# kasvii/GATOR

Hardware: AMD Instinct MI355X
Metric: meshes/sec (B=256, J=17) GATOR forward (higher is better)
Workload: dtype f32; 1 GPU; B=256 synthetic Human3.6M 17-joint poses per GPU, GAT+MDR forward fp32; batch_per_gpu=256, global_batch=256, num_joint=17, impl=fused, parallelism=dp1, mode=gather

## Files before the change

gator_amd/csrc/fused_common.h:

```cpp
#pragma once
#include <hip/hip_runtime.h>

namespace gator {

typedef float f32x16 __attribute__((ext_vector_type(16)));
typedef float f32x4 __attribute__((ext_vector_type(4)));

#define GATOR_MFMA(a, b, c) __builtin_amdgcn_mfma_f32_32x32x2f32((a), (b), (c), 0, 0, 0)

__device__ __forceinline__ int kap(int r) { return (r & 3) + 8 * (r >> 2); }

__device__ __forceinline__ f32x16 zero16() {
    f32x16 z;
#pragma unroll
    for (int r = 0; r < 16; ++r) z[r] = 0.f;
    return z;
}

struct HalfPair { float lo, hi; };
__device__ __forceinline__ HalfPair xhalves(float v) {
    const unsigned u = __float_as_uint(v);
    const auto r = __builtin_amdgcn_permlane32_swap(u, u, false, false);
    return HalfPair{__uint_as_float(r[0]), __uint_as_float(r[1])};
}
__device__ __forceinline__ float xhalf(float v) {
    const HalfPair q = xhalves(v);
    return (threadIdx.x & 32) ? q.lo : q.hi;
}

struct WTile { f32x4 g[4]; };

__device__ __forceinline__ WTile load_wtile(const float* __restrict__ Wp, int tile, int lane) {
    const f32x4* p = reinterpret_cast<const f32x4*>(Wp) + ((size_t)tile * 4) * 64 + lane;
    WTile t;
#pragma unroll
    for (int g = 0; g < 4; ++g) t.g[g] = p[g * 64];
    return t;
}

__device__ __forceinline__ f32x16 mma_T(const WTile& w, const f32x16& x, f32x16 acc) {
#pragma unroll
    for (int g = 0; g < 4; ++g)
#pragma unroll
        for (int j = 0; j < 4; ++j) acc = GATOR_MFMA(w.g[g][j], x[4 * g + j], acc);
    return acc;
}
__device__ __forceinline__ f32x16 mma_C(const WTile& w, const f32x16& x, f32x16 acc) {
#pragma unroll
    for (int g = 0; g < 4; ++g)
#pragma unroll
        for (int j = 0; j < 4; ++j) acc = GATOR_MFMA(x[4 * g + j], w.g[g][j], acc);
    return acc;
}

__device__ __forceinline__ void mma2_T(const WTile& w0, const f32x16& x0, f32x16& a0, const WTile& w1, const f32x16& x1, f32x16& a1) {
#pragma unroll
    for (int g = 0; g < 4; ++g)
#pragma unroll
        for (int j = 0; j < 4; ++j) {
            a0 = GATOR_MFMA(w0.g[g][j], x0[4 * g + j], a0);
            a1 = GATOR_MFMA(w1.g[g][j], x1[4 * g + j], a1);
        }
}
__device__ __forceinline__ void mma2_C(const WTile& w0, const f32x16& x0, f32x16& a0, const WTile& w1, const f32x16& x1, f32x16& a1) {
#pragma unroll
    for (int g = 0; g < 4; ++g)
#pragma unroll
        for (int j = 0; j < 4; ++j) {
            a0 = GATOR_MFMA(x0[4 * g + j], w0.g[g][j], a0);
            a1 = GATOR_MFMA(x1[4 * g + j], w1.g[g][j], a1);
        }
}
__device__ __forceinline__ f32x16 dot16(const f32x16& A, const f32x16& B, f32x16 init) {
    f32x16 e = init, o = zero16();
#pragma unroll
    for (int r = 0; r < 16; r += 2) {
        e = GATOR_MFMA(A[r], B[r], e);
        o = GATOR_MFMA(A[r + 1], B[r + 1], o);
    }
    return e + o;
}
__device__ __forceinline__ void dot16x2(const f32x16& A0, const f32x16& B0, f32x16& a0, const f32x16& A1, const f32x16& B1, f32x16& a1) {
#pragma unroll
    for (int r = 0; r < 16; ++r) {
        a0 = GATOR_MFMA(A0[r], B0[r], a0);
        a1 = GATOR_MFMA(A1[r], B1[r], a1);
    }
}

__device__ __forceinline__ f32x16 load_chanvec_T(const float* __restrict__ vec, int base, int h) {
    f32x16 v;
#pragma unroll
    for (int g = 0; g < 4; ++g) {
// ... 169 lines not shown
```

gator_amd/csrc/mdr_fused.hip:

```cpp
#include "fused_common.h"
#include "fused_state.h"
#include "x3_common.h"

#include <cmath>
#include <cstddef>
#include <cstdlib>
#include <type_traits>

namespace gator {
namespace {

constexpr float kLog2e = 1.4426950408889634f;

#ifdef GATOR_DIAG
__device__ int g_mdr_wmask = -1, g_mdr_kvmask = -1;
__device__ unsigned long long* g_persist_ends = nullptr;
#define MDR_WIDX(i) ((i) & g_mdr_wmask)
#define MDR_KVIDX(i) ((i) & g_mdr_kvmask)
#else
#define MDR_WIDX(i) (i)
#define MDR_KVIDX(i) (i)
#endif

struct LayerW {
// ... 136 lines not shown
    float m = -1e30f, l = 0.f;
    const float c = kLog2e * 0.17677669529663688110f;
#pragma unroll 1
    for (int kt = 0; kt < kVT - 2; kt += 4) {
        {
            const f32x16 kb = load_block(kbase + (size_t)kt * 2 * kTile, lane), vb = load_block(vbase + (size_t)kt * 2 * kTile, lane);
            ATTN_TILE(kt, kb, vb, O, O2)
        }
        {
            const f32x16 kb = load_block(kbase + (size_t)(kt + 1) * 2 * kTile, lane), vb = load_block(vbase + (size_t)(kt + 1) * 2 * kTile, lane);
            ATTN_TILE(kt + 1, kb, vb, O3, O4)
        }
        {
            const f32x16 kb = load_block(kbase + (size_t)(kt + 2) * 2 * kTile, lane), vb = load_block(vbase + (size_t)(kt + 2) * 2 * kTile, lane);
            ATTN_TILE(kt + 2, kb, vb, O, O2)
        }
        {
            const f32x16 kb = load_block(kbase + (size_t)(kt + 3) * 2 * kTile, lane), vb = load_block(vbase + (size_t)(kt + 3) * 2 * kTile, lane);
            ATTN_TILE(kt + 3, kb, vb, O3, O4)
        }
    }
    {
        const f32x16 kb = load_block(kbase + (size_t)(kVT - 2) * 2 * kTile, lane), vb = load_block(vbase + (size_t)(kVT - 2) * 2 * kTile, lane);
        ATTN_TILE(kVT - 2, kb, vb, O, O2)
    }
    {
        const f32x16 kb = load_block(kbase + (size_t)(kVT - 1) * 2 * kTile, lane), vb = load_block(vbase + (size_t)(kVT - 1) * 2 * kTile, lane);
        ATTN_TILE(kVT - 1, kb, vb, O3, O4)
    }
    l += xhalf(l);
    return ((O + O2) + (O3 + O4)) * (1.0f / l);
}

#define ATTN_TILE_X3(KT, KB, VB, OACC)                                                                      \
    {                                                                                                       \
        f32x16 S = x3_mma(KB, qx, zero16());                                           \
        float bm = -1e30f;                                                                                  \
        _Pragma("unroll") for (int r = 0; r < 16; ++r) {    \
            float sc = S[r];                                                                                \
            if ((KT) == kVT - 1 && kap(r) + 4 * h >= kV - 32 * (kVT - 1)) sc = -1e30f;                      \
            S[r] = sc;                                                                                      \
            bm = fmaxf(bm, sc);                                                                             \
        }                                                                                                   \
        bm = fmaxf(bm, xhalf(bm));                                                                          \
        if (!__all(bm <= m + 8.0f)) {                                                                       \
            const float mn = fmaxf(m, bm);                                                                  \
            const float al = __builtin_amdgcn_exp2f(m - mn);                                                \
            O = O * al;                                                                                     \
            O2 = O2 * al;                                                                                   \
            l *= al;                                                                                        \
            m = mn;                                                                                         \
        }                                                                                                   \
        float ps = 0.f;                                                                                     \
        _Pragma("unroll") for (int r = 0; r < 16; ++r) {                                                    \
            const float pe = __builtin_amdgcn_exp2f(S[r] - m);                                              \
            S[r] = pe;                                                                                      \
            ps += pe;                                                                                       \
        }                                                                                                   \
        l += ps;                                                                                            \
        OACC = x3_mma(VB, x3_split(S), OACC);             \
    }
__device__ __forceinline__ f32x16 self_attention_head_x3(const float* __restrict__ qt, const float* __restrict__ kbase,
                                                         const float* __restrict__ vbase, int lane) {
    const int h = lane >> 5;
    const X3 qx = x3_load(qt, lane);
    f32x16 O = zero16(), O2 = zero16();
    float m = -1e30f, l = 0.f;
    X3 kb = x3_load(kbase, lane), vb = x3_load(vbase, lane);
#pragma unroll 1
    for (int kt = 0; kt < kVT; kt += 2) {
        X3 kn = x3_load(kbase + (size_t)(kt + 1) * 2 * kTileX3, lane), vn = x3_load(vbase + (size_t)(kt + 1) * 2 * kTileX3, lane);
        ATTN_TILE_X3(kt, kb, vb, O)
        const int k2 = kt + 2 < kVT ? kt + 2 : kt;
        kb = x3_load(kbase + (size_t)k2 * 2 * kTileX3, lane);
        vb = x3_load(vbase + (size_t)k2 * 2 * kTileX3, lane);
        ATTN_TILE_X3(kt + 1, kn, vn, O2)
    }
    l += xhalf(l);
    return (O + O2) * (1.0f / l);
}

constexpr float kX2QK = 16.0f, kX2V = 16.0f;
#define ATTN_PV(VB, PX) { O2 = x2_mma_small(VB, PX, O2); O = x2_mma_main(VB, PX, O); }
#define ATTN_TILE_X2(KT, KB, VB)                                                                            \
    {                                                                                                       \
        MDR_PRIO_MFMA();                                                                                    \
        f32x16 S = x2_mma(KB, qx, zero16());                                     \
        MDR_PRIO_VALU();                                                                                    \
        float bm = -1e30f;                                                                                  \
        _Pragma("unroll") for (int r = 0; r < 16; ++r) {                                                    \
            float sc = S[r];                                                                                \
            if ((KT) == kVT - 1 && kap(r) + 4 * h >= kV - 32 * (kVT - 1)) sc = -1e30f;                      \
            S[r] = sc;                                                                                      \
            bm = fmaxf(bm, sc);                                                                             \
        }                                                                                                   \
        bm = fmaxf(bm, xhalf(bm));                                                                          \
        if (!__all(bm <= m + 2048.0f)) {                     \
            const float mn = fmaxf(m, bm);                                                                  \
            const float al = __builtin_amdgcn_exp2f((m - mn) * 0.00390625f);                                \
            O = O * al;                                                                                     \
            O2 = O2 * al;                                                                                   \
            l *= al;                                                                                        \
            m = mn;                                                                                         \
        }                                                                                                   \
        const float off = 6.0f - m * 0.00390625f;                                                           \
        float ps = 0.f;                                                                                     \
        _Pragma("unroll") for (int r = 0; r < 16; ++r) {                                                    \
            const float pe = __builtin_amdgcn_exp2f(fmaf(S[r], 0.00390625f, off));                          \
            S[r] = pe;                                                                                      \
            ps += pe;                                                                                       \
        }                                                                                                   \
        l += ps;                                                                                            \
        const X2 px_ = x2_split(S);                                                                         \
        MDR_PRIO_MFMA();                                                                                    \
                           \
        ATTN_PV(VB, px_)                                                                                    \
    }
template <bool kActScale16>
__device__ __forceinline__ f32x16 self_attention_head_x2(const float* __restrict__ qt, const float* __restrict__ kbase,
                                                         const float* __restrict__ vbase, int lane) {
    const int h = lane >> 5;
    const X2 qx = x2_load(qt, lane);
    f32x16 O = zero16(), O2 = zero16();
    float m = -1e30f, l = 0.f;
    X2 kb = x2_load(kbase, lane), vb = x2_load(vbase, lane);
#pragma unroll 1
    for (int kt = 0; kt < kVT - 2; kt += 2) {
        X2 kn = x2_load(kbase + (size_t)MDR_KVIDX(kt + 1) * 2 * kTile, lane), vn = x2_load(vbase + (size_t)MDR_KVIDX(kt + 1) * 2 * kTile, lane);
        ATTN_TILE_X2(0, kb, vb)
        kb = x2_load(kbase + (size_t)MDR_KVIDX(kt + 2) * 2 * kTile, lane);
        vb = x2_load(vbase + (size_t)MDR_KVIDX(kt + 2) * 2 * kTile, lane);
        ATTN_TILE_X2(0, kn, vn)
    }
    {
        X2 kn = x2_load(kbase + (size_t)MDR_KVIDX(kVT - 1) * 2 * kTile, lane), vn = x2_load(vbase + (size_t)MDR_KVIDX(kVT - 1) * 2 * kTile, lane);
        ATTN_TILE_X2(kVT - 2, kb, vb)
        ATTN_TILE_X2(kVT - 1, kn, vn)
    }
    l += xhalf(l);
    return (O + O2) * (((kActScale16 ? 16.0f : 1.0f) / kX2V) / l);
}


constexpr int kTileX1 = kTile / 2;
template <bool kActScale16>
__device__ __forceinline__ f32x16 self_attention_head_x1(const float* __restrict__ qt, const float* __restrict__ kbase,
                                                         const float* __restrict__ vbase, int lane) {
    const int h = lane >> 5;
    const X1 qx = x1_load(qt, lane);
    f32x16 O = zero16();
    float m = -1e30f, l = 0.f;
    X1 kA = x1_load(kbase, lane), vA = x1_load(vbase, lane);
    X1 kB = x1_load(kbase + (size_t)MDR_KVIDX(1) * 2 * kTileX1, lane), vB = x1_load(vbase + (size_t)MDR_KVIDX(1) * 2 * kTileX1, lane);
    f32x16 SA = x1_mma(kA, qx, zero16()), SB;
    float ci = 1e30f;
    auto step = [&](auto last_, const int kt, f32x16& Sc, f32x16& Sn, X1& Kc, const X1& Kn, X1& Vc) {
        constexpr int KT = decltype(last_)::value;
        if (KT != kVT - 1) Sn = x1_mma(Kn, qx, zero16());
        if (KT == kVT - 1) {
#pragma unroll
            for (int r = 0; r < 16; ++r) if (kap(r) + 4 * h >= kV - 32 * (kVT - 1)) Sc[r] = -1e30f;
        }
        float ps = 0.f;
        if (__all(ci < 1e29f)) {
#pragma unroll
            for (int r = 0; r < 16; ++r) { const float pe = __builtin_amdgcn_exp2f(Sc[r] + ci); ps += pe; Sc[r] = pe; }
        } else ps = 1e30f;
        if (!__all(ps < 32768.0f)) {
            f32x16 R = x1_mma(Kc, qx, zero16());
            float bm = -1e30f;
#pragma unroll
            for (int r = 0; r < 16; ++r) {
                if (KT == kVT - 1 && kap(r) + 4 * h >= kV - 32 * (kVT - 1)) R[r] = -1e30f;
                bm = fmaxf(bm, R[r]);
            }
            bm = fmaxf(bm, xhalf(bm));
            const float mn = fmaxf(m, bm);
            const float al = __builtin_amdgcn_exp2f(m - mn);
            O = O * al;
            l *= al;
            m = mn;
            ci = 6.0f - m;
            ps = 0.f;
#pragma unroll
            for (int r = 0; r < 16; ++r) { Sc[r] = __builtin_amdgcn_exp2f(R[r] + ci); ps += Sc[r]; }
        }
        l += ps;
        O = x1_mma(Vc, x1_cvt(Sc), O);
        __builtin_amdgcn_sched_barrier(0);
        if (kt + 2 < kVT) {
            Kc = x1_load(kbase + (size_t)MDR_KVIDX(kt + 2) * 2 * kTileX1, lane);
            Vc = x1_load(vbase + (size_t)MDR_KVIDX(kt + 2) * 2 * kTileX1, lane);
        }
        __builtin_amdgcn_sched_barrier(0);
    };
#pragma unroll 1
    for (int kt = 0; kt < kVT - 2; kt += 2) {
        step(std::integral_constant<int, 0>(), kt, SA, SB, kA, kB, vA);
        step(std::integral_constant<int, 0>(), kt + 1, SB, SA, kB, kA, vB);
    }
    step(std::integral_constant<int, 0>(), kVT - 2, SA, SB, kA, kB, vA);
    step(std::integral_constant<int, kVT - 1>(), kVT - 1, SB, SA, kB, kA, vB);
    l += xhalf(l);
    return O * (((kActScale16 ? 16.0f : 1.0f) / kX2V) / l);
}

__device__ __forceinline__ f32x16 cross_attention_head(const float* __restrict__ kj, const float* __restrict__ vjp,
                                                       const f32x16& qh, int J, int lane) {
    const int h = lane >> 5;
    const f32x16 kb = load_block(kj, lane);
    f32x16 S = dot16(kb, qh, zero16());
    const float c = kLog2e * 0.17677669529663688110f;
    float mx = -1e30f;
#pragma unroll
    for (int r = 0; r < 16; ++r) {
        const float s = (kap(r) + 4 * h < J) ? S[r] * c : -1e30f;
        S[r] = s;
        mx = fmaxf(mx, s);
    }
    mx = fmaxf(mx, xhalf(mx));
// ... 949 lines not shown
        float acc[3][3];
#pragma unroll
        for (int q = 0; q < 3; ++q) acc[q][0] = acc[q][1] = acc[q][2] = 0.f;
        int cch = lane / 3, ktap = lane - 3 * cch;
#pragma unroll(HOIST ? NIT : 1)
        for (int it = 0; it < NIT; ++it) {
            const int e = lane + 64 * it;
            if (e < kV * 3) {
                const float in0 = bn[cch][ktap], in1 = bn[cch][ktap + 1], in2 = bn[cch][ktap + 2];
#pragma unroll
                for (int q = 0; q < 3; ++q) {
                    const float w = HOIST ? wreg[q][HOIST ? it : 0] : conv_w(q, it);
                    acc[q][0] = fmaf(w, in0, acc[q][0]);
                    acc[q][1] = fmaf(w, in1, acc[q][1]);
                    acc[q][2] = fmaf(w, in2, acc[q][2]);
                }
            }
            cch += ktap == 2 ? 22 : 21;
            ktap = ktap == 2 ? 0 : ktap + 1;
        }
#pragma unroll
        for (int q = 0; q < 3; ++q)
#pragma unroll
            for (int l = 0; l < 3; ++l) {
                const double s = wave_sum64_f64((double)acc[q][l]);
                const int m = wave + NW * q;
                if (lane == 0 && m < 20) bc[m][l] = (float)(s + (double)a.bconv_b[m]);
            }
    }
    __syncthreads();
    const int mt = b >> 5, sl = b & 31;
    bool poisoned = false;
    if (a.persist_ctr) {
        int ch, b0, n;
        a.plan.locate(b, ch, b0, n);
        const unsigned* blk = a.persist_ctr + a.plan.block(ch);
        poisoned = blk[kCtrError] != 0u || blk[kCtrDone + (size_t)3 * n + (b - b0)] != (unsigned)kVT;
    }
    const float limit = a.vcp2 ? 4094.0f : 3.0e38f;
    bool bad = false;
    if (tok) {
        if (!HOIST) load_rows();
        float av[20];
#pragma unroll
        for (int g = 0; g < 5; ++g) { av[4 * g] = row[g][0]; av[4 * g + 1] = row[g][1]; av[4 * g + 2] = row[g][2]; av[4 * g + 3] = row[g][3]; }
        float mx = -1e30f, p[20], l = 0.f;
        for (int m = 0; m < 20; ++m) mx = fmaxf(mx, av[m]);
        for (int m = 0; m < 20; ++m) {
            p[m] = __builtin_amdgcn_exp2f((av[m] - mx) * kLog2e);
            l += p[m];
        }
        const float il = 1.0f / l;
        const float sc = a.alpha ? (float)exp((double)tail[3] * 0.09531017980432493) : 1.0f;
        const int cb = v >> 5, g = (v & 31) >> 3, hh = (v & 7) >> 2, j = v & 3;
        for (int c = 0; c < 3; ++c) {
            float o = 0.f;
            for (int m = 0; m < 20; ++m) o += (p[m] * il) * bc[m][c];
            float val = sc * o + cc[c];
            if (poisoned) val = __builtin_nanf("");
            bad = bad || !(fabsf(val) < limit);
            a.vc[((size_t)b * kV + v) * 3 + c] = val;
            if (a.vcp2) {
                const float sv = val * 16.0f;
                const _Float16 hi = (_Float16)sv;
                const _Float16 lo = (_Float16)(sv - (float)hi);
                const size_t pair = ((((size_t)(mt >> 2) * 28 + (v >> 4)) * 4 + (mt & 3)) * 3 + c) * 2;
                const size_t e = (size_t)(((v >> 3) & 1) * 32 + sl) * 8 + (v & 7);
                a.vcp2[pair * 512 + e] = hi; a.vcp2[(pair + 1) * 512 + e] = lo;
            } else if (a.vcp3) {
                const __bf16 hi = (__bf16)val;
                const float r1 = val - (float)hi;
                const __bf16 mid = (__bf16)r1;
                const __bf16 lo = (__bf16)(r1 - (float)mid);
                const size_t e = ((((size_t)mt * 3 + c) * 28 + (v >> 4)) * 64 + ((v >> 3) & 1) * 32 + sl) * 8 + (v & 7);
                a.vcp3[e] = hi; a.vcp3[a.vcp3_plane + e] = mid; a.vcp3[2 * a.vcp3_plane + e] = lo;
            } else {
                a.vcp[(((((size_t)mt * 3 + c) * kCB + cb) * 4 + g) * 64 + hh * 32 + sl) * 4 + j] = val;
            }
        }
    }
    head_report(a, b, bad, poisoned);
}

__global__ __launch_bounds__(256) void k_mdr_head_finish(const HeadArgs a, const double* __restrict__ hpart) {
    __shared__ float bc[20][3];
    const int b = blockIdx.x;
    bool poisoned = false;
    if (a.persist_ctr) {
        int ch, b0, n;
        a.plan.locate(b, ch, b0, n);
        const unsigned* blk = a.persist_ctr + a.plan.block(ch);
        poisoned = blk[kCtrError] != 0u || blk[kCtrDone + (size_t)3 * n + (b - b0)] != (unsigned)kVT;
    }
    head_finish<256>(a, hpart + (size_t)b * kVT * 64, b, poisoned, bc);
}

LayerW make_layer(const FusedState* f, const gator_ctx* c, int li) {
    const MdrLayerP& p = f->lay[li];
    const MdrLayerW& r = c->w.lay[li];
    LayerW w;
    auto sel = [&](const float* t) { return f->opt.mdr_x3 ? f->wxbuf + (size_t)(t - f->lay[0].wq) / kTile * kTileX3 : t; };
    w.wq = sel(p.wq); w.proj = sel(p.proj); w.fc1 = sel(p.fc1); w.fc2 = sel(p.fc2);
    w.sa0 = sel(p.sa[0]); w.sa1 = sel(p.sa[1]); w.sa2 = sel(p.sa[2]); w.sa3 = sel(p.sa[3]);
    w.n1w = r.n1w; w.n1b = r.n1b; w.proj_b = r.proj_b; w.n2w = r.n2w; w.n2b = r.n2b; w.fc1_b = r.fc1_b; w.fc2_b = r.fc2_b;
    w.a2 = r.a2; w.b2 = r.b2; w.sa0_b = r.sa_b[0]; w.sa1_b = r.sa_b[1]; w.sa2_b = r.sa_b[2]; w.sa3_b = r.sa_b[3];
    return w;
}

using MdrLayerKernel = void (*)(const MdrArgs, int);
using MdrPersistKernel = void (*)(const MdrPersistArgs);
constexpr MdrLayerKernel kMdrLayer[4][3] = {{k_mdr_layer<0, 3>, k_mdr_layer<1, 3>, k_mdr_layer<2, 3>}, {k_mdr_layer<0, 2>, k_mdr_layer<1, 2>, k_mdr_layer<2, 2>},
                                            {k_mdr_layer<0, 1>, k_mdr_layer<1, 1>, k_mdr_layer<2, 1>}, {k_mdr_layer<0, 0>, k_mdr_layer<1, 0>, k_mdr_layer<2, 0>}};
constexpr MdrPersistKernel kMdrPersist[4] = {k_mdr_persist<3>, k_mdr_persist<2>, k_mdr_persist<1>, k_mdr_persist<0>};

#ifdef GATOR_DIAG
struct MdrDiag { DevBuf<unsigned long long> st, ends; size_t solo = 0; };

int mdr_diag_setup(const FusedState* f, bool persist, hipStream_t st, MdrDiag& d) {
    static const int keep = -1, cut = 0;
    GATOR_HIP_CHECK(hipMemcpyToSymbolAsync(HIP_SYMBOL(g_mdr_wmask), (f->opt.mdr_cut & 1) ? &cut : &keep, sizeof(int), 0, hipMemcpyHostToDevice, st));
    GATOR_HIP_CHECK(hipMemcpyToSymbolAsync(HIP_SYMBOL(g_mdr_kvmask), (f->opt.mdr_cut & 2) ? &cut : &keep, sizeof(int), 0, hipMemcpyHostToDevice, st));
    d.solo = f->opt.mdr_solo ? 60 * 1024 : 0;
    if (f->opt.mdr_stamps) { GATOR_TRY(d.st.alloc(512 * sizeof(unsigned long long))); GATOR_HIP_CHECK(hipMemset(d.st, 0, 512 * sizeof(unsigned long long))); }
    if (f->opt.mdr_ends && persist) {
        GATOR_TRY(d.ends.alloc(3 * 1024 * sizeof(unsigned long long)));
        unsigned long long* d_ends = d.ends.get();
        GATOR_HIP_CHECK(hipMemset(d_ends, 0, 3 * 1024 * sizeof(unsigned long long)));
        GATOR_HIP_CHECK(hipMemcpyToSymbol(HIP_SYMBOL(g_persist_ends), &d_ends, sizeof(d_ends)));
    }
    return GATOR_OK;
}

int mdr_diag_report(MdrDiag& d, int B) {
    if (d.ends) {
        std::vector<unsigned long long> he(3 * 1024);
        GATOR_HIP_CHECK(hipMemcpy(he.data(), d.ends, he.size() * sizeof(unsigned long long), hipMemcpyDeviceToHost));
        unsigned long long* none = nullptr;
        GATOR_HIP_CHECK(hipMemcpyToSymbol(HIP_SYMBOL(g_persist_ends), &none, sizeof(none)));
        d.ends.reset();
        unsigned long long t0 = ~0ull, t1 = 0;
        int n = 0;
        for (int i = 0; i < 1024; ++i) if (he[3 * i + 2]) { t0 = std::min(t0, he[3 * i]); t1 = std::max(t1, he[3 * i + 2]); ++n; }
        if (n) {
            double idle = 0, lastlen = 0, first_end = 1e30, start_spread = 0;
            std::vector<double> ends;
            for (int i = 0; i < 1024; ++i) if (he[3 * i + 2]) {
                idle += (double)(t1 - he[3 * i + 2]) / 100.0;
                lastlen += (double)(he[3 * i + 2] - he[3 * i + 1]) / 100.0;
                first_end = std::min(first_end, (double)(he[3 * i + 2] - t0) / 100.0);
                start_spread = std::max(start_spread, (double)(he[3 * i] - t0) / 100.0);
                ends.push_back((double)(he[3 * i + 2] - t0) / 100.0);
            }
            std::sort(ends.begin(), ends.end());
            fprintf(stderr, "[k_mdr_persist ends, B=%d, %d workgroups] span %.1f us; workgroup starts spread over %.1f us; ends: first %.1f, p10 %.1f, median %.1f, p90 %.1f, last %.1f us; "
                            "mean idle before the last workgroup ends %.1f us; mean length of a workgroup's last stage-3 ticket %.1f us\n",
                    B, n, (double)(t1 - t0) / 100.0, start_spread, first_end, ends[n / 10], ends[n / 2], ends[n * 9 / 10], ends[n - 1], idle / n, lastlen / n);
        }
    }
    if (d.st) {
        unsigned long long hst[512];
        GATOR_HIP_CHECK(hipMemcpy(hst, d.st, sizeof(hst), hipMemcpyDeviceToHost));
        const int ns = (B * kVT + 63) / 64;
        unsigned long long t0 = ~0ull;
        for (int i = 0; i < ns && i < 120; ++i) if (hst[8 + 4 * i] && hst[8 + 4 * i] < t0) t0 = hst[8 + 4 * i];
        fprintf(stderr, "[k_mdr_layer<1> timeline, every 64th tile: tile:(start_us end_us kcycles xcc cu)]");
        for (int i = 0; i < ns && i < 120; ++i)
            fprintf(stderr, " %d:(%.0f,%.0f,%llu,x%llu,cu%llu.se%llu)", i * 64, (hst[8 + 4 * i] - t0) / 100.0, (hst[9 + 4 * i] - t0) / 100.0,
                    hst[10 + 4 * i] / 1000, hst[11 + 4 * i] >> 32, (hst[11 + 4 * i] >> 8) & 0xf, (hst[11 + 4 * i] >> 13) & 0x7);
        fprintf(stderr, "\n");
        d.st.reset();
        fprintf(stderr, "[k_mdr_layer<1> stamps, tile 0] attention(2 heads)=%llu outproj+res=%llu cross-attn block=%llu mlp=%llu customLN+qkv=%llu\n",
                hst[0], hst[1], hst[2], hst[3], hst[4]);
    }
    return GATOR_OK;
}
#endif

// ... 9 lines not shown
    ja.mdr_ctr = p.ctr_zero == CtrZero::MDR_JOINT ? ws.mdr_ctr : nullptr;
    ja.x2 = f->opt.mdr_x3 == 2;
    if (pc) {
        StageTimer tm(c, "mdr_joint", stream);
        k_mdr_joint<<<B, 128, 0, st>>>(ja);
    }
    const size_t per = (size_t)ws.cap * kVT * 2 * kTile;
    const size_t perq = (size_t)ws.cap * kVT * 2 * (f->opt.mdr_x3 == 1 ? kTileX3 : kTile);
    float* set[3][4] = {{ws.vf, ws.q, ws.k, ws.v}, {ws.vf + per, ws.q + perq, ws.k + perq, ws.v + perq},
                        {ws.vf + 2 * per, ws.q + 2 * perq, ws.k + 2 * perq, ws.v + 2 * perq}};
    MdrArgs a{};
    a.B = B; a.J = c->J; a.jkv = ws.jkv; a.pc = pc; a.xout = pc ? nullptr : x_out; a.vj = w.vj; a.tok_base = f->tok_base; a.tok_w3 = f->tok_w3;
    a.head_w = f->opt.mdr_x3 ? f->wxbuf + (size_t)(f->head_w - f->lay[0].wq) / kTile * kTileX3 : f->head_w; a.head_b = f->head_b; a.hf = ws.hf; a.lbf = c->block_taps ? ws.lbf : nullptr;
    a.hpart = p.head == MdrHead::FINISH ? reinterpret_cast<double*>(ws.hpart) : nullptr;
    a.bconv_w = w.bconv_w; a.hbn_w = w.bn_w; a.hbn_b = w.bn_b; a.hbn_mean = w.bn_mean; a.hbn_var = w.bn_var; a.halpha = c->alpha;
    a.lin_s = f->opt.mdr_x3 == 2 ? std::ldexp(kActScale, f->mdr_wshift) : 1.0f;
    a.lin_inv = 1.0f / a.lin_s;
    const int nwg = (B * kVT + 3) / 4;
#ifdef GATOR_DIAG
    MdrDiag diag;
    GATOR_TRY(mdr_diag_setup(f, persist, st, diag));
    const size_t solo = xa != 0 ? diag.solo : 0;
#else
    constexpr size_t solo = 0;
#endif
    MdrPersistArgs pa{};
    for (int li = 0; li <= 3; ++li) {
#ifdef GATOR_DIAG
        a.stamps = (li == 1) ? diag.st.get() : nullptr;
#endif
        float** in = persist ? set[(li + 2) % 3] : set[(li + 1) & 1];
        float** out = persist ? set[li % 3] : set[li & 1];
        a.layer = li;
        a.vf_in = in[0]; a.q_in = in[1]; a.k_in = in[2]; a.v_in = in[3];
        a.vf_out = out[0]; a.q_out = out[1]; a.k_out = out[2]; a.v_out = out[3];
        if (li > 0) a.prev = make_layer(f, c, li - 1);
        if (li < 3) a.cur = make_layer(f, c, li);
        if (persist) { pa.st[li] = a; continue; }
        StageTimer tm(c, li == 0 ? "mdr_layer0" : (li < 3 ? "mdr_layer" : "mdr_attn_head"), stream);
        const MdrLayerKernel layer = kMdrLayer[3 - xa][li == 0 ? 0 : li < 3 ? 1 : 2];
        layer<<<nwg, 256, li < 3 ? solo : 0, st>>>(a, nwg);
    }
    if (persist) {
        StageTimer tm(c, "mdr_layers", stream);
        const size_t tq = f->opt.mdr_x3 == 1 ? kTileX3 : (xa == 3 ? kTileX1 : kTile);
        for (int ch = 0, b0 = 0; ch < p.chunks.nch; ++ch) {
            const int n = p.chunks.base + (ch < p.chunks.rem ? 1 : 0);
            MdrPersistArgs pc_ = pa;
            for (int li = 0; li <= 3; ++li) {
                MdrArgs& s = pc_.st[li];
                const size_t ov = (size_t)b0 * kVT * 2 * kTile, oq = (size_t)b0 * kVT * 2 * tq;
                s.B = n;
                s.vf_in += ov; s.q_in += oq; s.k_in += oq; s.v_in += oq;
                s.vf_out += ov; s.q_out += oq; s.k_out += oq; s.v_out += oq;
                s.jkv += (size_t)b0 * 12 * kTile;
                if (s.pc) s.pc += (size_t)b0 * c->J * 133;
                if (s.xout) s.xout += (size_t)b0 * c->J * 3;
                s.hf += (size_t)b0 * kV * 32;
                if (s.hpart) s.hpart += (size_t)b0 * kVT * 64;
                if (s.lbf) s.lbf += (size_t)b0 * kV * kE;
            }
            pc_.ctr = ws.mdr_ctr + p.chunks.block(ch);
            const MdrPersistKernel layers = kMdrPersist[3 - xa];
            layers<<<p.grid, 256, 0, st>>>(pc_);
            b0 += n;
        }
    }
#ifdef GATOR_DIAG
    GATOR_TRY(mdr_diag_report(diag, B));
#endif
    HeadArgs ha;
    ha.hf = ws.hf; ha.bn_w = w.bn_w; ha.bn_b = w.bn_b; ha.bn_mean = w.bn_mean; ha.bn_var = w.bn_var;
    ha.bconv_w = w.bconv_w; ha.bconv_b = w.bconv_b; ha.vc = ws.vc; ha.vcp = ws.vcp;
    ha.persist_ctr = persist ? ws.mdr_ctr : nullptr;
    ha.plan = p.chunks;
    ha.status = c->status_dev;
    ha.pose2d = pose2d; ha.J = c->J;
    ha.vcp2 = f->opt.up_x3 == 2 ? (_Float16*)ws.vcp3 : nullptr;
    ha.vcp3 = f->opt.up_x3 == 1 ? (__bf16*)ws.vcp3 : nullptr; ha.vcp3_plane = upsample_x3_vcp_elems(ws.cap) / 3;
    ha.alpha = c->alpha;
    {
        StageTimer tm(c, "mdr_head", stream);
        switch (p.head) {
        case MdrHead::FINISH: k_mdr_head_finish<<<B, 256, 0, st>>>(ha, a.hpart); break;
        case MdrHead::WHOLE_HOIST: k_mdr_head<512, true><<<B, 512, 0, st>>>(ha); break;
        case MdrHead::WHOLE: k_mdr_head<512, false><<<B, 512, 0, st>>>(ha); break;
        }
    }
    GATOR_HIP_CHECK(hipGetLastError());
    c->set_tap(TAP_MDR_LBF2, c->block_taps ? ws.lbf : nullptr, c->block_taps ? (int64_t)B * kV * kE : 0);
    c->set_tap(TAP_VERT431, ws.vc, (int64_t)B * kV * 3);
    return GATOR_OK;
}

}
```

gator_amd/csrc/upsample_x2.hip:

```cpp
#include <cmath>
#include <cstring>

#include "upsample_common.h"

namespace gator {
namespace {

constexpr int kNBuf = 4, kStageFrags = 36;
constexpr int kActShift = 4;

__device__ __forceinline__ void split2(float x, _Float16& h, _Float16& l) {
    h = (_Float16)x;
    l = (_Float16)(x - (float)h);
}

__global__ void k_pack_up_x2(const float* __restrict__ w, _Float16* __restrict__ dst, int64_t n_frag_pairs, float scale) {
    const int64_t e = (int64_t)blockIdx.x * blockDim.x + threadIdx.x;
    if (e >= n_frag_pairs * 512) return;
    const int j = e & 7, lane = (e >> 3) & 63;
    int64_t r = e >> 9;
    const int tap = r % 3; r /= 3;
    const int o2 = r & 1; r >>= 1;
    const int s = r % kS16;
    const int op = (int)(r / kS16);
    const int o = 32 * (2 * op + o2) + (lane & 31), c = 16 * s + 8 * (lane >> 5) + j;
    const float x = (o < kNV && c < kV) ? w[((int64_t)o * kV + c) * 3 + tap] * scale : 0.f;
    _Float16 h, l;
    split2(x, h, l);
    const int64_t pair = (((int64_t)op * kS16 + s) * 2 + o2) * 3 + tap;
    dst[(pair * 2 + 0) * 512 + lane * 8 + j] = h;
    dst[(pair * 2 + 1) * 512 + lane * 8 + j] = l;
}
__global__ void k_pack_vc_x2(const float* __restrict__ vc, int B, _Float16* __restrict__ ap, int64_t n_frag_pairs) {
    const int64_t e = (int64_t)blockIdx.x * blockDim.x + threadIdx.x;
    if (e >= n_frag_pairs * 512) return;
    const int j = e & 7, lane = (e >> 3) & 63;
    int64_t r = e >> 9;
    const int lp = r % 3; r /= 3;
    const int mi = r & 3; r >>= 2;
    const int s = r % kS16;
    const int mg = (int)(r / kS16);
    const int smp = 32 * (4 * mg + mi) + (lane & 31), c = 16 * s + 8 * (lane >> 5) + j;
    const float x = (smp < B && c < kV) ? vc[((int64_t)smp * kV + c) * 3 + lp] * (float)(1 << kActShift) : 0.f;
    _Float16 h, l;
    split2(x, h, l);
    const int64_t pair = (((int64_t)mg * kS16 + s) * 4 + mi) * 3 + lp;
    ap[(pair * 2 + 0) * 512 + lane * 8 + j] = h;
    ap[(pair * 2 + 1) * 512 + lane * 8 + j] = l;
}

__global__ void k_absmax(const float* __restrict__ w, int64_t n, unsigned* __restrict__ out) {
    float m = 0.f;
    for (int64_t i = (int64_t)blockIdx.x * blockDim.x + threadIdx.x; i < n; i += (int64_t)gridDim.x * blockDim.x) {
        const float a = fabsf(w[i]);
        m = a > m || a != a ? a : m;
    }
    for (int o = 32; o > 0; o >>= 1) {
        const float q = __shfl_xor(m, o);
        m = q > m || q != q ? q : m;
    }
    if ((threadIdx.x & 63) == 0) atomicMax(out, __float_as_uint(m));
}

__device__ __forceinline__ void dma_frag(const void* base, unsigned lane_off, unsigned lds_dst) {
    unsigned keep;
    asm volatile("s_mov_b32 %0, m0\n\ts_mov_b32 m0, %3\n\ts_nop 0\n\tglobal_load_lds_dwordx4 %1, %2\n\ts_mov_b32 m0, %0"
                 : "=&s"(keep) : "v"(lane_off), "s"(base), "s"(lds_dst) : "memory");
}
template <int N> __device__ __forceinline__ void wait_vm() { asm volatile("s_waitcnt vmcnt(%0)" ::"n"(N) : "memory"); }

template <bool WLO = true>
__global__ __launch_bounds__(512, 1) void k_upsample_x2(const _Float16* __restrict__ ap, const _Float16* __restrict__ wp,
                                                        const float* __restrict__ bias, const float* __restrict__ tpl,
                                                        float* __restrict__ out, int B, int MT, int MG, int nwg, float unscale,
                                                        const JregEpi jr) {
    extern __shared__ __attribute__((aligned(16))) unsigned char lds_raw[];
    f16x8 (*st)[kStageFrags][64] = reinterpret_cast<f16x8 (*)[kStageFrags][64]>(lds_raw);
    const int lane = threadIdx.x & 63, wave = __builtin_amdgcn_readfirstlane(threadIdx.x >> 6);
    const int wg = xcd_remap(blockIdx.x, nwg);
    const int obp = wg / MG, mg = wg % MG;
    const int mi = wave & 3, oi = wave >> 2;
    const int ob = 2 * obp + oi, mt = 4 * mg + mi;
    const bool live = mt < MT;
    const unsigned lane_off = lane * 16;
    const unsigned lds0 = (unsigned)(unsigned long long)lds_raw;
    const char* a_src = reinterpret_cast<const char*>(ap) + (size_t)mg * kS16 * 24 * 1024;
    const char* w_src = reinterpret_cast<const char*>(wp) + (size_t)obp * kS16 * 12 * 1024;
    const char* src[5];
    unsigned stride[5], dsto[5];
#pragma unroll
    for (int i = 0; i < 5; ++i) {
        const int f = wave + 8 * i;
        src[i] = f < 24 ? a_src + f * 1024 : w_src + (f - 24) * 1024;
        stride[i] = f < 24 ? 24 * 1024 : 12 * 1024;
        dsto[i] = lds0 + f * 1024;
    }
    auto issue = [&](int s) {
        const unsigned dst = (unsigned)(s & (kNBuf - 1)) * kStageFrags * 1024;
#pragma unroll
        for (int i = 0; i < 4; ++i) dma_frag(src[i] + (size_t)s * stride[i], lane_off, dst + dsto[i]);
        if (wave < 4) dma_frag(src[4] + (size_t)s * stride[4], lane_off, dst + dsto[4]);
    };
    auto wait_landed = [&](int younger) {
        if (younger >= 1) { if (wave < 4) wait_vm<5>(); else wait_vm<4>(); }
        else wait_vm<0>();
    };
    f32x16 big[3], sm[3], tot[3];
#pragma unroll
    for (int l = 0; l < 3; ++l) { big[l] = zero16(); sm[l] = zero16(); tot[l] = zero16(); }
    f16x8 a[3][2], w[3][2];
    auto load_first = [&](int s) {
        const f16x8 (*cur)[64] = st[s & (kNBuf - 1)];
#pragma unroll
        for (int p = 0; p < 2; ++p) {
            a[0][p] = cur[mi * 6 + p][lane];
            w[0][p] = cur[24 + oi * 6 + p][lane];
            w[1][p] = cur[24 + oi * 6 + 2 + p][lane];
        }
    };
    auto load_rest = [&](int s) {
        const f16x8 (*cur)[64] = st[s & (kNBuf - 1)];
#pragma unroll
        for (int p = 0; p < 2; ++p) {
            a[1][p] = cur[mi * 6 + 2 + p][lane];
            w[2][p] = cur[24 + oi * 6 + 4 + p][lane];
            a[2][p] = cur[mi * 6 + 4 + p][lane];
        }
    };
    issue(0); issue(1); issue(2);
    if (wave < 4) wait_vm<10>(); else wait_vm<8>();
    __builtin_amdgcn_s_barrier();
    load_first(0);
#pragma unroll 1
    for (int s = 0; s < kS16; ++s) {
        if (s + 1 < kS16) wait_landed(kS16 - 2 - s);
        __builtin_amdgcn_s_barrier();
        if (s + 3 < kS16) issue(s + 3);
        load_rest(s);
        if (live) {
#pragma unroll
            for (int lp = 0; lp < 3; ++lp)
#pragma unroll
                for (int k = 2; k >= 0; --k) {
                    const int l = lp + 1 - k;
                    if (l < 0 || l > 2) continue;
                    big[l] = GATOR_MFMA_F16(a[lp][0], w[k][0], big[l]);
                    if constexpr (WLO) sm[l] = GATOR_MFMA_F16(a[lp][0], w[k][1], sm[l]);
                    sm[l] = GATOR_MFMA_F16(a[lp][1], w[k][0], sm[l]);
                }
            if (s % 7 == 6) {
#pragma unroll
                for (int l = 0; l < 3; ++l) { tot[l] += big[l]; big[l] = zero16(); }
            }
        }
        if (s + 1 < kS16) load_first(s + 1);
    }
    const int ov = 32 * ob + (lane & 31), h = lane >> 5;
    if (ov >= kNV || !live) return;
    const float bo = bias[ov];
    const float t0 = tpl[ov * 3], t1 = tpl[ov * 3 + 1], t2 = tpl[ov * 3 + 2];
    const int2 jb = jr.P ? jr.blk[ob] : int2{0, 0};
#pragma unroll
    for (int r = 0; r < 16; ++r) {
        const int smp = 32 * mt + kap(r) + 4 * h;
        if (smp < B) {
            F3 v;
            v.x = ((tot[0][r] + sm[0][r]) * unscale + bo) + t0;
            v.y = ((tot[1][r] + sm[1][r]) * unscale + bo) + t1;
            v.z = ((tot[2][r] + sm[2][r]) * unscale + bo) + t2;
            if (out) *reinterpret_cast<F3*>(out + ((int64_t)smp * kNV + ov) * 3) = v;
            for (int e = jb.x; e < jb.x + jb.y; ++e) {
                const int2 en = jr.ent[e];
                if (en.x == ov) {
                    const float we = jr.w[e];
                    F3 q;
                    q.x = we * v.x; q.y = we * v.y; q.z = we * v.z;
                    *reinterpret_cast<F3*>(jr.P + ((int64_t)smp * jr.nnz + en.y) * 3) = q;
                }
            }
        }
    }
}

constexpr size_t kX2Lds = (size_t)kNBuf * kStageFrags * 1024;

}

size_t upsample_x2_weight_elems() { return (size_t)(kOB / 2) * kS16 * 12 * 512; }
size_t upsample_x2_vcp_elems(int B) { return (size_t)((B + 127) / 128) * kS16 * 24 * 512; }

int upsample_x2_prepare_device() {
    GATOR_HIP_CHECK(hipFuncSetAttribute((const void*)k_upsample_x2<true>, hipFuncAttributeMaxDynamicSharedMemorySize, (int)kX2Lds));
    GATOR_HIP_CHECK(hipFuncSetAttribute((const void*)k_upsample_x2<false>, hipFuncAttributeMaxDynamicSharedMemorySize, (int)kX2Lds));
    return GATOR_OK;
}

int pack_upsample_x2(const float* up_w, void* dst, float* unscale, void* stream) {
    hipStream_t st = (hipStream_t)stream;
    DevBuf<unsigned> d_max;
    GATOR_TRY(d_max.alloc(sizeof(unsigned)));
    GATOR_HIP_CHECK(hipMemsetAsync(d_max, 0, sizeof(unsigned), st));
    const int64_t n = (int64_t)kNV * kV * 3;
    k_absmax<<<1024, 256, 0, st>>>(up_w, n, d_max.get());
    unsigned bits = 0;
    GATOR_HIP_CHECK(hipMemcpyAsync(&bits, d_max, sizeof(unsigned), hipMemcpyDeviceToHost, st));
    GATOR_HIP_CHECK(hipStreamSynchronize(st));
    d_max.reset();
    float wmax;
    static_assert(sizeof(wmax) == sizeof(bits), "float bits");
    memcpy(&wmax, &bits, sizeof(wmax));
    int shift = 0;
    if (wmax > 0.f && std::isfinite(wmax)) {
        int e;
        (void)std::frexp(wmax, &e);
        shift = 14 - e;
        if (shift > 118) shift = 118;
        if (shift < -118) shift = -118;
    }
    const int64_t pairs = (int64_t)upsample_x2_weight_elems() / 1024;
    k_pack_up_x2<<<(unsigned)((pairs * 512 + 255) / 256), 256, 0, st>>>(up_w, (_Float16*)dst, pairs, std::ldexp(1.0f, shift));
    GATOR_HIP_CHECK(hipGetLastError());
    *unscale = std::ldexp(1.0f, -(shift + kActShift));
    return GATOR_OK;
}

int launch_pack_vc_x2(const float* vc, int B, void* vcp2, void* stream) {
    const int64_t pairs = (int64_t)upsample_x2_vcp_elems(B) / 1024;
    k_pack_vc_x2<<<(unsigned)((pairs * 512 + 255) / 256), 256, 0, (hipStream_t)stream>>>(vc, B, (_Float16*)vcp2, pairs);
    GATOR_HIP_CHECK(hipGetLastError());
    return GATOR_OK;
}

int launch_upsample_x2(const FusedState* f, const gator_ctx* c, const FusedWs& ws, int B, float* verts, void* stream, bool with_joints, bool w1) {
    const int MT = (B + 31) / 32, MG = (MT + 3) / 4;
    const JregEpi jr = jreg_epi(f, with_joints);
    const int nwg = (kOB / 2) * MG;
    if (w1) k_upsample_x2<false><<<nwg, 512, kX2Lds, (hipStream_t)stream>>>((const _Float16*)ws.vcp3, (const _Float16*)f->up_w2.get(), c->w.up_b, c->w.v6890,
                                                                           verts, B, MT, MG, nwg, f->up_w2_unscale, jr);
// ... 8 lines not shown
```

Baseline: 447,200 meshes/sec.

## Trim masked work in last attention tile, skip padded upsample steps, widen head finish

The attention loop now gives the final key tile its own routine. It handles only the score registers that can hold live keys, and it issues three f16 MFMAs for PV instead of the full split product. The per-register mask check is removed from every other tile. The upsample GEMM loop now stops at the k-step count needed to cover the live columns rather than the padded kS16, with a final accumulation of the partial sums added. The head-finish kernel block size goes from 256 to 512 threads.

```diff
diff --git a/gator_amd/csrc/fused_common.h b/gator_amd/csrc/fused_common.h
--- a/gator_amd/csrc/fused_common.h
+++ b/gator_amd/csrc/fused_common.h
@@ -8,7 +8,7 @@
 
 #define GATOR_MFMA(a, b, c) __builtin_amdgcn_mfma_f32_32x32x2f32((a), (b), (c), 0, 0, 0)
 
-__device__ __forceinline__ int kap(int r) { return (r & 3) + 8 * (r >> 2); }
+__host__ __device__ __forceinline__ constexpr int kap(int r) { return (r & 3) + 8 * (r >> 2); }
 
 __device__ __forceinline__ f32x16 zero16() {
     f32x16 z;
diff --git a/gator_amd/csrc/mdr_fused.hip b/gator_amd/csrc/mdr_fused.hip
--- a/gator_amd/csrc/mdr_fused.hip
+++ b/gator_amd/csrc/mdr_fused.hip
@@ -242,18 +242,14 @@
 
 constexpr float kX2QK = 16.0f, kX2V = 16.0f;
 #define ATTN_PV(VB, PX) { O2 = x2_mma_small(VB, PX, O2); O = x2_mma_main(VB, PX, O); }
-#define ATTN_TILE_X2(KT, KB, VB)                                                                            \
+#define ATTN_TILE_X2(KB, VB)                                                                                \
     {                                                                                                       \
         MDR_PRIO_MFMA();                                                                                    \
         f32x16 S = x2_mma(KB, qx, zero16());                                     \
         MDR_PRIO_VALU();                                                                                    \
         float bm = -1e30f;                                                                                  \
-        _Pragma("unroll") for (int r = 0; r < 16; ++r) {                                                    \
-            float sc = S[r];                                                                                \
-            if ((KT) == kVT - 1 && kap(r) + 4 * h >= kV - 32 * (kVT - 1)) sc = -1e30f;                      \
-            S[r] = sc;                                                                                      \
-            bm = fmaxf(bm, sc);                                                                             \
-        }                                                                                                   \
+        _Pragma("unroll") for (int r = 0; r < 16; ++r)                                                      \
+            bm = fmaxf(bm, S[r]);                                                                           \
         bm = fmaxf(bm, xhalf(bm));                                                                          \
         if (!__all(bm <= m + 2048.0f)) {                     \
             const float mn = fmaxf(m, bm);                                                                  \
@@ -276,6 +272,53 @@
                            \
         ATTN_PV(VB, px_)                                                                                    \
     }
+constexpr int kLastTileKeys = kV - 32 * (kVT - 1);
+constexpr bool last_tile_kstep1_is_masked() {
+    for (int r = 8; r < 16; ++r)
+        if (kap(r) < kLastTileKeys) return false;
+    for (int r = 0; r < 8; ++r)
+        if (kap(r) + 4 >= 16) return false;
+    return true;
+}
+static_assert(kLastTileKeys > 0 && kLastTileKeys <= 16 && last_tile_kstep1_is_masked(),
+              "ATTN_TILE_X2_LAST skips score registers 8..15: every key they hold must be masked");
+#define ATTN_TILE_X2_LAST(KB, VB)                                                                           \
+    {                                                                                                       \
+        MDR_PRIO_MFMA();                                                                                    \
+        f32x16 S = x2_mma(KB, qx, zero16());                                                                \
+        MDR_PRIO_VALU();                                                                                    \
+        float bm = -1e30f;                                                                                  \
+        _Pragma("unroll") for (int r = 0; r < 8; ++r) {                                                     \
+            float sc = S[r];                                                                                \
+            if (kap(r) + 4 * h >= kLastTileKeys) sc = -1e30f;           \
+            S[r] = sc;                                                                                      \
+            bm = fmaxf(bm, sc);                                                                             \
+        }                                                                                                   \
+        bm = fmaxf(bm, xhalf(bm));                                                                          \
+        if (!__all(bm <= m + 2048.0f)) {                                                                    \
+            const float mn = fmaxf(m, bm);                                                                  \
+            const float al = __builtin_amdgcn_exp2f((m - mn) * 0.00390625f);                                \
+            O = O * al;                                                                                     \
+            O2 = O2 * al;                                                                                   \
+            l *= al;                                                                                        \
+            m = mn;                                                                                         \
+        }                                                                                                   \
+        const float off = 6.0f - m * 0.00390625f;                                                           \
+        float ps = 0.f;                                                                                     \
+        f16x8 ph_, pl_;                                                                                     \
+        _Pragma("unroll") for (int r = 0; r < 8; ++r) {                                                     \
+            const float pe = __builtin_amdgcn_exp2f(fmaf(S[r], 0.00390625f, off));                          \
+            ps += pe;                                                                                       \
+            const _Float16 hi_ = (_Float16)pe;                                      \
+            ph_[r] = hi_;                                                                                   \
+            pl_[r] = (_Float16)(pe - (float)hi_);                                                           \
+        }                                                                                                   \
+        l += ps;                                                                                            \
+        MDR_PRIO_MFMA();                                                                                    \
+        O2 = GATOR_MFMA_F16(VB.p[1][0], ph_, O2);                               \
+        O2 = GATOR_MFMA_F16(VB.p[0][0], pl_, O2);                                                           \
+        O = GATOR_MFMA_F16(VB.p[0][0], ph_, O);                                  \
+    }
 template <bool kActScale16>
 __device__ __forceinline__ f32x16 self_attention_head_x2(const float* __restrict__ qt, const float* __restrict__ kbase,
                                                          const float* __restrict__ vbase, int lane) {
@@ -287,15 +330,15 @@
 #pragma unroll 1
     for (int kt = 0; kt < kVT - 2; kt += 2) {
         X2 kn = x2_load(kbase + (size_t)MDR_KVIDX(kt + 1) * 2 * kTile, lane), vn = x2_load(vbase + (size_t)MDR_KVIDX(kt + 1) * 2 * kTile, lane);
-        ATTN_TILE_X2(0, kb, vb)
+        ATTN_TILE_X2(kb, vb)
         kb = x2_load(kbase + (size_t)MDR_KVIDX(kt + 2) * 2 * kTile, lane);
         vb = x2_load(vbase + (size_t)MDR_KVIDX(kt + 2) * 2 * kTile, lane);
-        ATTN_TILE_X2(0, kn, vn)
+        ATTN_TILE_X2(kn, vn)
     }
     {
         X2 kn = x2_load(kbase + (size_t)MDR_KVIDX(kVT - 1) * 2 * kTile, lane), vn = x2_load(vbase + (size_t)MDR_KVIDX(kVT - 1) * 2 * kTile, lane);
-        ATTN_TILE_X2(kVT - 2, kb, vb)
-        ATTN_TILE_X2(kVT - 1, kn, vn)
+        ATTN_TILE_X2(kb, vb)
+        ATTN_TILE_X2_LAST(kn, vn)
     }
     l += xhalf(l);
     return (O + O2) * (((kActScale16 ? 16.0f : 1.0f) / kX2V) / l);
@@ -1411,7 +1454,8 @@
     head_report(a, b, bad, poisoned);
 }
 
-__global__ __launch_bounds__(256) void k_mdr_head_finish(const HeadArgs a, const double* __restrict__ hpart) {
+constexpr int kHeadFinishNT = 512;
+__global__ __launch_bounds__(kHeadFinishNT) void k_mdr_head_finish(const HeadArgs a, const double* __restrict__ hpart) {
     __shared__ float bc[20][3];
     const int b = blockIdx.x;
     bool poisoned = false;
@@ -1421,7 +1465,7 @@
         const unsigned* blk = a.persist_ctr + a.plan.block(ch);
         poisoned = blk[kCtrError] != 0u || blk[kCtrDone + (size_t)3 * n + (b - b0)] != (unsigned)kVT;
     }
-    head_finish<256>(a, hpart + (size_t)b * kVT * 64, b, poisoned, bc);
+    head_finish<kHeadFinishNT>(a, hpart + (size_t)b * kVT * 64, b, poisoned, bc);
 }
 
 LayerW make_layer(const FusedState* f, const gator_ctx* c, int li) {
@@ -1597,7 +1641,7 @@
     {
         StageTimer tm(c, "mdr_head", stream);
         switch (p.head) {
-        case MdrHead::FINISH: k_mdr_head_finish<<<B, 256, 0, st>>>(ha, a.hpart); break;
+        case MdrHead::FINISH: k_mdr_head_finish<<<B, kHeadFinishNT, 0, st>>>(ha, a.hpart); break;
         case MdrHead::WHOLE_HOIST: k_mdr_head<512, true><<<B, 512, 0, st>>>(ha); break;
         case MdrHead::WHOLE: k_mdr_head<512, false><<<B, 512, 0, st>>>(ha); break;
         }
diff --git a/gator_amd/csrc/upsample_x2.hip b/gator_amd/csrc/upsample_x2.hip
--- a/gator_amd/csrc/upsample_x2.hip
+++ b/gator_amd/csrc/upsample_x2.hip
@@ -8,6 +8,9 @@
 
 constexpr int kNBuf = 4, kStageFrags = 36;
 constexpr int kActShift = 4;
+constexpr int kSteps = (kV + 15) / 16;
+static_assert(kSteps <= kS16 && 16 * kSteps >= kV, "every live column is inside a k-step that runs");
+static_assert(kSteps >= 3, "the prologue issues three stages");
 
 __device__ __forceinline__ void split2(float x, _Float16& h, _Float16& l) {
     h = (_Float16)x;
@@ -132,10 +135,10 @@
     __builtin_amdgcn_s_barrier();
     load_first(0);
 #pragma unroll 1
-    for (int s = 0; s < kS16; ++s) {
-        if (s + 1 < kS16) wait_landed(kS16 - 2 - s);
+    for (int s = 0; s < kSteps; ++s) {
+        if (s + 1 < kSteps) wait_landed(kSteps - 2 - s);
         __builtin_amdgcn_s_barrier();
-        if (s + 3 < kS16) issue(s + 3);
+        if (s + 3 < kSteps) issue(s + 3);
         load_rest(s);
         if (live) {
 #pragma unroll
@@ -153,7 +156,11 @@
                 for (int l = 0; l < 3; ++l) { tot[l] += big[l]; big[l] = zero16(); }
             }
         }
-        if (s + 1 < kS16) load_first(s + 1);
+        if (s + 1 < kSteps) load_first(s + 1);
+    }
+    if (live) {
+#pragma unroll
+        for (int l = 0; l < 3; ++l) tot[l] += big[l];
     }
     const int ov = 32 * ob + (lane & 31), h = lane >> 5;
     if (ov >= kNV || !live) return;
```

Result: no change. 450,100 meshes/sec, median of 6 (+0.6%).
